# xandercai/JSPSR

Measured on AMD Instinct MI355X. Metric: Mpixels/sec fwd+bwd, JSPSR x8 on 512^2 DEM tiles, higher is better.
Workload: dtype bf16; 1 GPU; jspsr_r8_img_msk (image+mask guided, 43.87M params), 8 x 512x512 tiles per GPU, train step (fwd + L1/L2/Sobel loss + bwd + grad all-reduce + AdamW); storage policy: bf16 activations / gradients / MFMA operands, fp32 accumulation, BatchNorm statistics, master weights and optimizer, and the generator head (affinity logits + offsets) kept as fp32 planes; tiles_per_gpu=8, tile=512, global_tiles=8, parallelism=dp1, step_mode=eager

## Files before the change

jspsr_amd/csrc/elementwise.hip:

```cpp
#include "common.h"

#include <cstdlib>

namespace {

using namespace jspsr;

constexpr int TX = 64, TY = 4;

template <typename T> struct V;
template <> struct V<float> { static constexpr int N = 4; };
template <> struct V<__bf16> { static constexpr int N = 8; };

template <typename T, int N>
struct Pack { T v[N]; };

template <typename T>
__device__ __forceinline__ uint4 load_raw(const T* p) { return *reinterpret_cast<const uint4*>(p); }
template <typename T>
__device__ __forceinline__ void unpack(const uint4& raw, float (&f)[V<T>::N]) {
  if constexpr (sizeof(T) == 4) {
    f[0] = __uint_as_float(raw.x); f[1] = __uint_as_float(raw.y); f[2] = __uint_as_float(raw.z); f[3] = __uint_as_float(raw.w);
  } else {
    const unsigned w[4] = {raw.x, raw.y, raw.z, raw.w};
// ... 514 lines not shown
    for (int k = 0; k < 8; ++k) {
      const size_t o = ((size_t)b * chunks + r + k) * C + c;
      ps[k] = psum[o]; pm[k] = pmax[o]; pi[k] = pidx[o];
    }
#pragma unroll
    for (int k = 0; k < 8; ++k) {
      s += (double)ps[k];
      if (pm[k] > m || (pm[k] == m && pi[k] < ii)) { m = pm[k]; ii = pi[k]; }
    }
  }
  for (; r < chunks; ++r) {
    const size_t o = ((size_t)b * chunks + r) * C + c;
    s += (double)psum[o];
    if (pmax[o] > m || (pmax[o] == m && pidx[o] < ii)) { m = pmax[o]; ii = pidx[o]; }
  }
  avg[(size_t)b * C + c] = (float)(s / (double)npix);
  mx[(size_t)b * C + c] = m;
  amax[(size_t)b * C + c] = ii;
}

template <typename T>
__global__ __launch_bounds__(TX * TY) void gate_scale_kernel(const T* __restrict__ x, const float* __restrict__ s,
                                                            T* __restrict__ y, RedGeom g) {
  constexpr int N = V<T>::N;
  float sv[N];
  const int c0 = lane_map<N>(g).c;
  if (c0 < g.C) load_param<N>(s + (size_t)(blockIdx.x / g.chunks) * g.C + c0, sv);
  for_pixels_mlp<T, 1>(
      g, [&](long long pix, int c, uint4 (&raw)[1]) { raw[0] = load_raw<T>(x + (size_t)pix * g.C + c); },
      [&](long long, long long pix, int c, const uint4 (&raw)[1]) {
        float f[N];
        unpack<T>(raw[0], f);
#pragma unroll
        for (int k = 0; k < N; ++k) f[k] *= sv[k];
        store_vec<T>(y + (size_t)pix * g.C + c, f);
      });
}

template <typename T>
__global__ __launch_bounds__(TX * TY) void gate_bwd_reduce_kernel(const T* __restrict__ dy, const T* __restrict__ x,
                                                                 RedGeom g, float* __restrict__ partial) {
  constexpr int N = V<T>::N;
  reduce_pixels_mlp<T, 1, 2>(
      g, partial,
      [&](long long pix, int c, uint4 (&raw)[2]) {
        raw[0] = load_raw<T>(dy + (size_t)pix * g.C + c);
        raw[1] = load_raw<T>(x + (size_t)pix * g.C + c);
      },
      [&](long long, int, const uint4 (&raw)[2], float (&acc)[1][N]) {
        float d[N], xv[N];
        unpack<T>(raw[0], d);
        unpack<T>(raw[1], xv);
#pragma unroll
        for (int i = 0; i < N; ++i) acc[0][i] += d[i] * xv[i];
      });
}

__global__ void gate_bwd_finalize_kernel(const float* __restrict__ partial, int chunks, int C, float* __restrict__ ds) {
  const int c = blockIdx.x * blockDim.x + threadIdx.x, b = blockIdx.y;
  if (c >= C) return;
  double s = 0.0;
  int r = 0;
  for (; r + 8 <= chunks; r += 8) {
    float v[8];
#pragma unroll
    for (int k = 0; k < 8; ++k) v[k] = partial[((size_t)b * chunks + r + k) * C + c];
#pragma unroll
    for (int k = 0; k < 8; ++k) s += (double)v[k];
  }
  for (; r < chunks; ++r) s += (double)partial[((size_t)b * chunks + r) * C + c];
  ds[(size_t)b * C + c] = (float)s;
}

template <typename T>
__global__ __launch_bounds__(TX * TY) void gate_bwd_apply_kernel(const T* __restrict__ dy, const float* __restrict__ s,
                                                                const float* __restrict__ davg, const float* __restrict__ dmax,
                                                                const int* __restrict__ amax, T* __restrict__ dx, RedGeom g) {
  constexpr int N = V<T>::N;
  float sv[N], da[N], dm[N];
  int am[N];
  const int c0 = lane_map<N>(g).c;
  const float inv = 1.f / (float)g.npix;
  if (c0 < g.C) {
    const size_t o = (size_t)(blockIdx.x / g.chunks) * g.C + c0;
    load_param<N>(s + o, sv); load_param<N>(davg + o, da); load_param<N>(dmax + o, dm);
#pragma unroll
    for (int k = 0; k < N; ++k) { am[k] = amax[o + k]; da[k] *= inv; }
  }
  for_pixels_mlp<T, 1>(
      g, [&](long long pix, int c, uint4 (&raw)[1]) { raw[0] = load_raw<T>(dy + (size_t)pix * g.C + c); },
      [&](long long p, long long pix, int c, const uint4 (&raw)[1]) {
        float f[N];
        unpack<T>(raw[0], f);
#pragma unroll
        for (int k = 0; k < N; ++k) f[k] = f[k] * sv[k] + da[k] + (am[k] == (int)p ? dm[k] : 0.f);
        store_vec<T>(dx + (size_t)pix * g.C + c, f);
      });
}

int ew_blocks(long long total) {
  long long b = (total + 255) / 256;
  return (int)(b < 1 ? 1 : (b > 4096 ? 4096 : b));
}

int check_c(int dtype, int C, const char* what) {
  if (dtype != JSPSR_F32 && dtype != JSPSR_BF16) return fail(JSPSR_EINVAL, "%s: bad dtype", what);
  const int vec = dtype == JSPSR_F32 ? 4 : 8;
  if (C <= 0 || C % vec) return fail(JSPSR_EINVAL, "%s: C=%d must be a multiple of %d", what, C, vec);
  return JSPSR_OK;
}

}

#define DISPATCH(dtype, CALL)                    \
  do {                                           \
    if ((dtype) == JSPSR_F32) { using T = float; CALL; } else { using T = __bf16; CALL; } \
  } while (0)

extern "C" size_t jspsr_reduce_workspace_bytes(int dtype, int C, int nseg) {
  if (C <= 0 || nseg <= 0) return 0;
  const int vec = dtype == JSPSR_F32 ? 4 : 8;
  const RedGeom g = make_red(1LL << 40, nseg, C, vec);
  const size_t rows = (size_t)nseg * g.chunks;
  return (rows * 3 + 4) * (size_t)C * sizeof(float) + 64;
}

extern "C" int jspsr_bn_forward(int dtype, const void* x, int x_cs, int x_coff, const void* res, int r_cs, int r_coff,
                                void* y, int y_cs, int y_coff, const float* gamma, const float* beta,
                                float* running_mean, float* running_var, float momentum, float eps, int training,
                                int relu, float res_scale, float* save_mean, float* save_invstd, long long npix, int C,
                                const float* ext_partial, int ext_rows, const float* res_affine, float* affine_out,
                                void* workspace, jspsr_stream_t stream) {
  if (int e = check_c(dtype, C, "bn_forward")) return e;
  if (!x || (!y && !affine_out) || !gamma || !beta || !save_mean || !save_invstd || !workspace || npix <= 0)
    return fail(JSPSR_EINVAL, "bn_forward: null pointer or empty tensor");
  if (res_affine && !res) return fail(JSPSR_EINVAL, "bn_forward: res_affine without a residual operand");
  if (!training && (!running_mean || !running_var)) return fail(JSPSR_EINVAL, "bn_forward: eval mode needs running stats");
  const int vec = dtype == JSPSR_F32 ? 4 : 8;
  if (x_cs % vec || x_coff % vec || y_cs % vec || y_coff % vec || (res && (r_cs % vec || r_coff % vec)))
    return fail(JSPSR_EINVAL, "bn_forward: channel pitches/offsets must be multiples of %d", vec);
  hipStream_t s = static_cast<hipStream_t>(stream);
  float* ws = static_cast<float*>(workspace);
  float* scale = affine_out ? affine_out : ws;
  float* shift = affine_out ? affine_out + C : ws + C;
  float* partial = ws + 2 * C;
  int rows = 0;
  if (training && ext_partial) {
    if (ext_rows <= 0) return fail(JSPSR_EINVAL, "bn_forward: ext_rows must be positive");
    rows = ext_rows < 256 ? ext_rows : 256;
    if (ext_rows > 256) {
      hipLaunchKernelGGL(fold_rows_kernel, dim3(rows, (2 * C + 255) / 256), dim3(256), 0, s, ext_partial, ext_rows, 2 * C, rows, partial);
      if (int e = check_launch("bn_fold_rows")) return e;
    } else {
      (void)hipMemcpyAsync(partial, ext_partial, (size_t)ext_rows * 2 * C * sizeof(float), hipMemcpyDeviceToDevice, s);
    }
  } else if (training) {
    const RedGeom g = make_red(npix, 1, C, vec);
    rows = g.chunks;
    DISPATCH(dtype, hipLaunchKernelGGL(bn_stats_kernel<T>, red_grid(g, vec), dim3(TX, TY), 0, s,
                                       static_cast<const T*>(x), x_cs, x_coff, g, partial));
    if (int e = check_launch("bn_stats")) return e;
  }
  hipLaunchKernelGGL(bn_finalize_kernel, dim3((C + 3) / 4), dim3(256), 0, s, partial, rows, C, npix, gamma, beta,
                     running_mean, running_var, momentum, eps, training, save_mean, save_invstd, scale, shift);
  if (int e = check_launch("bn_finalize")) return e;
  if (!y) return JSPSR_OK;
  const RedGeom ga = make_red(npix, 1, C, vec);
#define BN_APPLY(R) DISPATCH(dtype, hipLaunchKernelGGL((bn_apply_kernel<T, R>), red_grid(ga, vec), dim3(TX, TY), 0, s,             \
                                     static_cast<const T*>(x), x_cs, x_coff, static_cast<const T*>(res), r_cs, r_coff,        \
                                     static_cast<T*>(y), y_cs, y_coff, scale, shift, res_affine, res_scale, relu, ga))
  if (res) { BN_APPLY(true); } else { BN_APPLY(false); }
#undef BN_APPLY
  return check_launch("bn_apply");
}

__global__ void bn_reduce_params_kernel(const float* __restrict__ gamma, const float* __restrict__ beta, const float* __restrict__ mean,
                                        const float* __restrict__ invstd, int C, float* __restrict__ par) {
  const int c = blockIdx.x * blockDim.x + threadIdx.x;
  if (c >= C) return;
  const float a = gamma[c] * invstd[c];
  par[c] = a;
  par[C + c] = beta[c] - a * mean[c];
  par[2 * C + c] = invstd[c];
  par[3 * C + c] = -mean[c] * invstd[c];
}

extern "C" int jspsr_bn_reduce_params(const float* gamma, const float* beta, const float* save_mean, const float* save_invstd, int C,
                                      float* par, jspsr_stream_t stream) {
  if (!gamma || !beta || !save_mean || !save_invstd || !par || C <= 0) return fail(JSPSR_EINVAL, "bn_reduce_params: bad arguments");
  hipLaunchKernelGGL(bn_reduce_params_kernel, dim3((C + 255) / 256), dim3(256), 0, static_cast<hipStream_t>(stream), gamma, beta,
                     save_mean, save_invstd, C, par);
  return check_launch("bn_reduce_params");
}

extern "C" int jspsr_bn_backward(int dtype, const void* dy, int dy_cs, int dy_coff, const void* y, int y_cs, int y_coff,
                                 const void* x, int x_cs, int x_coff, const float* gamma, const float* beta, const float* save_mean,
                                 const float* save_invstd, int training, int relu, float res_scale, void* dx, void* dres,
                                 float* dgamma, float* dbeta, int accumulate, long long npix, int C, void* workspace,
                                 const float* ext_partial, int ext_rows, jspsr_stream_t stream) {
  if (int e = check_c(dtype, C, "bn_backward")) return e;
  if (!dy || !x || !gamma || !save_mean || !save_invstd || !dx || !dgamma || !dbeta || !workspace || npix <= 0 ||
      (relu == 1 && !y) || (relu == 2 && !beta) || relu < 0 || relu > 2)
    return fail(JSPSR_EINVAL, "bn_backward: null pointer, empty tensor or bad relu mode");
  const int vec = dtype == JSPSR_F32 ? 4 : 8;
  if (dy_cs % vec || dy_coff % vec || x_cs % vec || x_coff % vec || (relu == 1 && (y_cs % vec || y_coff % vec)))
    return fail(JSPSR_EINVAL, "bn_backward: channel pitches/offsets must be multiples of %d", vec);
  hipStream_t s = static_cast<hipStream_t>(stream);
  float* ws = static_cast<float*>(workspace);
  float* coef = ws;
  float* partial = ws + 3 * C;
  const RedGeom g = make_red(npix, 1, C, vec);
#define BN_BWD_REDUCE(R) DISPATCH(dtype, hipLaunchKernelGGL((bn_bwd_reduce_kernel<T, R>), red_grid(g, vec), dim3(TX, TY), 0, s, \
                                     static_cast<const T*>(dy), dy_cs, dy_coff, static_cast<const T*>(y), y_cs, y_coff,     \
                                     static_cast<const T*>(x), x_cs, x_coff, save_mean, save_invstd, gamma, beta, g, partial))
  int rows = g.chunks;
  if (ext_partial) {
    if (ext_rows <= 0) return fail(JSPSR_EINVAL, "bn_backward: ext_rows must be positive");
    if (ext_rows > 1024) {
      rows = g.chunks < 1024 ? (g.chunks > 0 ? g.chunks : 1) : 1024;
      hipLaunchKernelGGL(fold_rows_kernel, dim3(rows, (2 * C + 255) / 256), dim3(256), 0, s, ext_partial, ext_rows, 2 * C, rows, partial);
      if (int e = check_launch("bn_fold_rows")) return e;
    } else {
      partial = const_cast<float*>(ext_partial);
      rows = ext_rows;
    }
  } else {
    if (relu == 0) { BN_BWD_REDUCE(0); } else if (relu == 1) { BN_BWD_REDUCE(1); } else { BN_BWD_REDUCE(2); }
    if (int e = check_launch("bn_bwd_reduce")) return e;
  }
#undef BN_BWD_REDUCE
  hipLaunchKernelGGL(bn_bwd_finalize_kernel, dim3((C + 3) / 4), dim3(256), 0, s, partial, rows, C, npix, gamma,
                     save_invstd, training, res_scale, accumulate, dgamma, dbeta, coef);
  if (int e = check_launch("bn_bwd_finalize")) return e;
#define BN_BWD_APPLY(R) DISPATCH(dtype, hipLaunchKernelGGL((bn_bwd_apply_kernel<T, R>), red_grid(g, vec), dim3(TX, TY), 0, s,  \
                                     static_cast<const T*>(dy), dy_cs, dy_coff, static_cast<const T*>(y), y_cs, y_coff,     \
                                     static_cast<const T*>(x), x_cs, x_coff, save_mean, save_invstd, gamma, beta, coef,     \
                                     static_cast<T*>(dx), static_cast<T*>(dres), g))
  if (relu == 0) { BN_BWD_APPLY(0); } else if (relu == 1) { BN_BWD_APPLY(1); } else { BN_BWD_APPLY(2); }
#undef BN_BWD_APPLY
  return check_launch("bn_bwd_apply");
}

extern "C" int jspsr_bn_fold(const float* gamma, const float* beta, const float* running_mean, const float* running_var,
                             float eps, float res_scale, int C, float* scale, float* shift, jspsr_stream_t stream) {
  if (!gamma || !beta || !running_mean || !running_var || !scale || !shift || C <= 0)
    return fail(JSPSR_EINVAL, "bn_fold: bad arguments");
  hipLaunchKernelGGL(bn_fold_kernel, dim3((C + 255) / 256), dim3(256), 0, static_cast<hipStream_t>(stream), gamma, beta,
                     running_mean, running_var, eps, res_scale, C, scale, shift);
  return check_launch("bn_fold");
}

extern "C" int jspsr_act_backward(int dtype, const void* dy, int dy_cs, int dy_coff, const void* y, int y_cs, int relu,
                                  void* dz, int dz_cs, float* dbias, long long npix, int C, void* workspace,
                                  jspsr_stream_t stream) {
  if (int e = check_c(dtype, C, "act_backward")) return e;
  if (!dy || (relu && !y) || !workspace || npix <= 0) return fail(JSPSR_EINVAL, "act_backward: null pointer or empty tensor");
  const int vec = dtype == JSPSR_F32 ? 4 : 8;
  if (dy_cs % vec || dy_coff % vec || (dz && dz_cs % vec) || (relu && (y_cs % vec || y_cs < C)))
    return fail(JSPSR_EINVAL, "act_backward: bad pitch");
  hipStream_t s = static_cast<hipStream_t>(stream);
  float* partial = static_cast<float*>(workspace);
  const RedGeom g = make_red(npix, 1, C, vec);
#define ACT_BWD(R) DISPATCH(dtype, hipLaunchKernelGGL((act_bwd_kernel<T, R>), red_grid(g, vec), dim3(TX, TY), 0, s, static_cast<const T*>(dy), \
                                     dy_cs, dy_coff, static_cast<const T*>(y), y_cs, relu, static_cast<T*>(dz), dz_cs, g, partial))
  if (relu) { ACT_BWD(true); } else { ACT_BWD(false); }
#undef ACT_BWD
  if (int e = check_launch("act_backward")) return e;
  if (dbias) {
    hipLaunchKernelGGL(sum_rows_kernel, dim3((C + 3) / 4), dim3(256), 0, s, partial, g.chunks, 1, 0, C, dbias);
    return check_launch("act_backward_bias");
  }
  return JSPSR_OK;
}

extern "C" int jspsr_gate_pool(int dtype, const void* x, int B, long long npix, int C, float* avg, float* mx, int* amax,
                               void* workspace, jspsr_stream_t stream) {
  if (int e = check_c(dtype, C, "gate_pool")) return e;
  if (!x || !avg || !mx || !amax || !workspace || B <= 0 || npix <= 0 || npix > 0x7fffffffLL)
    return fail(JSPSR_EINVAL, "gate_pool: bad arguments");
  const int vec = dtype == JSPSR_F32 ? 4 : 8;
  hipStream_t s = static_cast<hipStream_t>(stream);
  const RedGeom g = make_red(npix, B, C, vec);
  const size_t rows = (size_t)B * g.chunks;
  float* psum = static_cast<float*>(workspace);
  float* pmax = psum + rows * C;
  int* pidx = reinterpret_cast<int*>(pmax + rows * C);
  DISPATCH(dtype, hipLaunchKernelGGL(gate_pool_kernel<T>, red_grid(g, vec), dim3(TX, TY), 0, s, static_cast<const T*>(x), g,
                                     psum, pmax, pidx));
  if (int e = check_launch("gate_pool")) return e;
  hipLaunchKernelGGL(gate_pool_finalize_kernel, dim3((C + 255) / 256, B), dim3(256), 0, s, psum, pmax, pidx, g.chunks, C,
                     npix, avg, mx, amax);
  return check_launch("gate_pool_finalize");
}

extern "C" int jspsr_gate_scale(int dtype, const void* x, const float* s_, void* y, int B, long long npix, int C,
                                jspsr_stream_t stream) {
  if (int e = check_c(dtype, C, "gate_scale")) return e;
  if (!x || !s_ || !y || B <= 0 || npix <= 0) return fail(JSPSR_EINVAL, "gate_scale: bad arguments");
  const int vec = dtype == JSPSR_F32 ? 4 : 8;
  hipStream_t s = static_cast<hipStream_t>(stream);
  const RedGeom g = make_red(npix, B, C, vec);
  DISPATCH(dtype, hipLaunchKernelGGL(gate_scale_kernel<T>, red_grid(g, vec), dim3(TX, TY), 0, s,
                                     static_cast<const T*>(x), s_, static_cast<T*>(y), g));
  return check_launch("gate_scale");
}

extern "C" int jspsr_gate_backward_reduce(int dtype, const void* dy, const void* x, float* ds, int B, long long npix, int C,
                                          void* workspace, jspsr_stream_t stream) {
  if (int e = check_c(dtype, C, "gate_backward_reduce")) return e;
  if (!dy || !x || !ds || !workspace || B <= 0 || npix <= 0) return fail(JSPSR_EINVAL, "gate_backward_reduce: bad arguments");
  const int vec = dtype == JSPSR_F32 ? 4 : 8;
  hipStream_t s = static_cast<hipStream_t>(stream);
  const RedGeom g = make_red(npix, B, C, vec);
  float* partial = static_cast<float*>(workspace);
  DISPATCH(dtype, hipLaunchKernelGGL(gate_bwd_reduce_kernel<T>, red_grid(g, vec), dim3(TX, TY), 0, s,
                                     static_cast<const T*>(dy), static_cast<const T*>(x), g, partial));
  if (int e = check_launch("gate_backward_reduce")) return e;
  hipLaunchKernelGGL(gate_bwd_finalize_kernel, dim3((C + 255) / 256, B), dim3(256), 0, s, partial, g.chunks, C, ds);
  return check_launch("gate_backward_finalize");
}

extern "C" int jspsr_gate_backward_apply(int dtype, const void* dy, const float* s_, const float* davg, const float* dmax,
                                         const int* amax, void* dx, int B, long long npix, int C, jspsr_stream_t stream) {
  if (int e = check_c(dtype, C, "gate_backward_apply")) return e;
  if (!dy || !s_ || !davg || !dmax || !amax || !dx || B <= 0 || npix <= 0)
    return fail(JSPSR_EINVAL, "gate_backward_apply: bad arguments");
  const int vec = dtype == JSPSR_F32 ? 4 : 8;
  hipStream_t s = static_cast<hipStream_t>(stream);
  const RedGeom g = make_red(npix, B, C, vec);
  DISPATCH(dtype, hipLaunchKernelGGL(gate_bwd_apply_kernel<T>, red_grid(g, vec), dim3(TX, TY), 0, s,
                                     static_cast<const T*>(dy), s_, davg, dmax, amax, static_cast<T*>(dx), g));
  return check_launch("gate_backward_apply");
}

template <typename T>
__global__ __launch_bounds__(256) void nchw_to_nhwc_kernel(const float* __restrict__ src, T* __restrict__ dst, int C, long long HW,
                                                          long long npix, int Cpad) {
  constexpr int N = V<T>::N;
  for (long long p = blockIdx.x * 256LL + threadIdx.x; p < npix; p += (long long)gridDim.x * 256) {
    const long long b = p / HW, q = p - b * HW;
    const float* s = src + (size_t)b * C * HW + q;
    T* d = dst + (size_t)p * Cpad;
    for (int c0 = 0; c0 < Cpad; c0 += N) {
      float f[N];
#pragma unroll
      for (int i = 0; i < N; ++i) f[i] = c0 + i < C ? s[(size_t)(c0 + i) * HW] : 0.f;
      store_vec<T>(d + c0, f);
    }
  }
}

extern "C" int jspsr_nchw_to_nhwc(int dtype, const float* src, void* dst, int B, int C, int H, int W, int c_pad,
                                  jspsr_stream_t stream) {
  if (dtype != JSPSR_F32 && dtype != JSPSR_BF16) return fail(JSPSR_EINVAL, "nchw_to_nhwc: dtype must be JSPSR_F32 or JSPSR_BF16");
  const int vec = dtype == JSPSR_F32 ? 4 : 8;
  if (!src || !dst || B <= 0 || C <= 0 || H <= 0 || W <= 0 || c_pad < C || c_pad % vec)
    return fail(JSPSR_EINVAL, "nchw_to_nhwc: bad arguments (c_pad must be a multiple of %d and >= C)", vec);
  if (!aligned4(src) || !aligned16(dst)) return fail(JSPSR_EALIGN, "nchw_to_nhwc: src must be 4-byte, dst 16-byte aligned");
  const long long HW = (long long)H * W, npix = HW * B;
  const long long want = (npix + 255) / 256;
  const int blocks = (int)(want > 8192 ? 8192 : want);
  hipStream_t s = static_cast<hipStream_t>(stream);
  DISPATCH(dtype, hipLaunchKernelGGL(nchw_to_nhwc_kernel<T>, dim3(blocks), dim3(256), 0, s, src, static_cast<T*>(dst), C, HW, npix, c_pad));
  return check_launch("nchw_to_nhwc");
}

constexpr int GM_T = 256;

__global__ __launch_bounds__(GM_T) void gate_mlp_fwd_kernel(const float* __restrict__ avg, const float* __restrict__ mx,
                                                           const float* __restrict__ w1, const float* __restrict__ w2, int C, int Ch,
                                                           float* __restrict__ s, float* __restrict__ hid) {
  extern __shared__ float gm_lds[];
  const int b = blockIdx.x, tid = threadIdx.x, wave = tid >> 6, lane = tid & 63;
  const float* a = avg + (size_t)b * C;
  const float* m = mx + (size_t)b * C;
  for (int j = wave; j < Ch; j += GM_T / 64) {
    const float* w = w1 + (size_t)j * C;
    float da = 0.f, dm = 0.f;
    for (int c = lane; c < C; c += 64) { const float wv = w[c]; da += wv * a[c]; dm += wv * m[c]; }
#pragma unroll
    for (int d = 32; d > 0; d >>= 1) { da += __shfl_xor(da, d, 64); dm += __shfl_xor(dm, d, 64); }
    if (lane == 0) {
      const float ha = fmaxf(da, 0.f), hm = fmaxf(dm, 0.f);
      hid[((size_t)b * 2 + 0) * Ch + j] = ha;
      hid[((size_t)b * 2 + 1) * Ch + j] = hm;
      gm_lds[j] = ha + hm;
    }
  }
  __syncthreads();
  for (int c = tid; c < C; c += GM_T) {
    const float* w = w2 + (size_t)c * Ch;
    float z = 0.f;
    for (int j = 0; j < Ch; ++j) z += w[j] * gm_lds[j];
    s[(size_t)b * C + c] = 1.f / (1.f + expf(-z));
  }
}

__global__ __launch_bounds__(GM_T) void gate_mlp_bwd_kernel(const float* __restrict__ ds, const float* __restrict__ s,
                                                           const float* __restrict__ hid, const float* __restrict__ w1,
                                                           const float* __restrict__ w2, int C, int Ch, float* __restrict__ davg,
                                                           float* __restrict__ dmax, float* __restrict__ dzs, float* __restrict__ dhs) {
  extern __shared__ float gm_lds[];
  float* dz = gm_lds;
  float* dh = gm_lds + C;
  const int b = blockIdx.x, tid = threadIdx.x, wave = tid >> 6, lane = tid & 63;
  for (int c = tid; c < C; c += GM_T) {
    const float sv = s[(size_t)b * C + c], v = ds[(size_t)b * C + c] * sv * (1.f - sv);
    dz[c] = v;
    dzs[(size_t)b * C + c] = v;
  }
  __syncthreads();
  for (int j = wave; j < Ch; j += GM_T / 64) {
    float acc = 0.f;
    for (int c = lane; c < C; c += 64) acc += w2[(size_t)c * Ch + j] * dz[c];
#pragma unroll
    for (int d = 32; d > 0; d >>= 1) acc += __shfl_xor(acc, d, 64);
    if (lane == 0) {
      const float da = hid[((size_t)b * 2 + 0) * Ch + j] > 0.f ? acc : 0.f, dm = hid[((size_t)b * 2 + 1) * Ch + j] > 0.f ? acc : 0.f;
      dh[j] = da; dh[Ch + j] = dm;
      dhs[((size_t)b * 2 + 0) * Ch + j] = da;
      dhs[((size_t)b * 2 + 1) * Ch + j] = dm;
    }
  }
  __syncthreads();
  for (int c = tid; c < C; c += GM_T) {
    float ga = 0.f, gm = 0.f;
    for (int j = 0; j < Ch; ++j) { const float wv = w1[(size_t)j * C + c]; ga += wv * dh[j]; gm += wv * dh[Ch + j]; }
    davg[(size_t)b * C + c] = ga;
    dmax[(size_t)b * C + c] = gm;
  }
}

__global__ __launch_bounds__(GM_T) void gate_mlp_wgrad_kernel(const float* __restrict__ dzs, const float* __restrict__ dhs,
                                                             const float* __restrict__ hid, const float* __restrict__ avg,
                                                             const float* __restrict__ mx, int B, int C, int Ch,
                                                             float* __restrict__ dw1, float* __restrict__ dw2) {
  const long long n = (long long)C * Ch;
  for (long long i = blockIdx.x * (long long)GM_T + threadIdx.x; i < 2 * n; i += (long long)gridDim.x * GM_T) {
    if (i < n) {
      const int j = (int)(i / C), c = (int)(i - (long long)j * C);
      float g = 0.f;
      for (int b = 0; b < B; ++b)
        g += dhs[((size_t)b * 2 + 0) * Ch + j] * avg[(size_t)b * C + c] + dhs[((size_t)b * 2 + 1) * Ch + j] * mx[(size_t)b * C + c];
      dw1[i] = g;
    } else {
      const long long k = i - n;
      const int c = (int)(k / Ch), j = (int)(k - (long long)c * Ch);
      float g = 0.f;
      for (int b = 0; b < B; ++b) g += dzs[(size_t)b * C + c] * (hid[((size_t)b * 2 + 0) * Ch + j] + hid[((size_t)b * 2 + 1) * Ch + j]);
      dw2[k] = g;
    }
  }
}

extern "C" int jspsr_gate_mlp_forward(const float* avg, const float* mx, const float* w1, const float* w2, int B, int C, int Ch,
                                      float* s, float* hid, jspsr_stream_t stream) {
  if (!avg || !mx || !w1 || !w2 || !s || !hid || B <= 0 || C <= 0 || Ch <= 0 || Ch > 4096)
    return fail(JSPSR_EINVAL, "gate_mlp_forward: bad arguments");
  hipLaunchKernelGGL(gate_mlp_fwd_kernel, dim3(B), dim3(GM_T), Ch * sizeof(float), static_cast<hipStream_t>(stream), avg, mx, w1, w2,
                     C, Ch, s, hid);
  return check_launch("gate_mlp_forward");
}

extern "C" size_t jspsr_gate_mlp_backward_workspace_bytes(int B, int C, int Ch) {
  if (B <= 0 || C <= 0 || Ch <= 0) return 0;
  return ((size_t)B * C + (size_t)B * 2 * Ch) * sizeof(float);
}

extern "C" int jspsr_gate_mlp_backward(const float* ds, const float* s, const float* hid, const float* avg, const float* mx,
                                       const float* w1, const float* w2, int B, int C, int Ch, float* davg, float* dmax,
                                       float* dw1, float* dw2, void* workspace, jspsr_stream_t stream) {
  if (!ds || !s || !hid || !avg || !mx || !w1 || !w2 || !davg || !dmax || !dw1 || !dw2 || !workspace || B <= 0 || C <= 0 ||
      Ch <= 0 || (size_t)(C + 2 * Ch) * sizeof(float) > 64 * 1024)
    return fail(JSPSR_EINVAL, "gate_mlp_backward: bad arguments");
  float* dzs = static_cast<float*>(workspace);
  float* dhs = dzs + (size_t)B * C;
  hipStream_t st = static_cast<hipStream_t>(stream);
  hipLaunchKernelGGL(gate_mlp_bwd_kernel, dim3(B), dim3(GM_T), (C + 2 * Ch) * sizeof(float), st, ds, s, hid, w1, w2, C, Ch, davg, dmax,
                     dzs, dhs);
  if (int e = check_launch("gate_mlp_backward")) return e;
  const long long n2 = 2LL * C * Ch;
  const int blocks = (int)((n2 + GM_T - 1) / GM_T > 2048 ? 2048 : (n2 + GM_T - 1) / GM_T);
  hipLaunchKernelGGL(gate_mlp_wgrad_kernel, dim3(blocks), dim3(GM_T), 0, st, dzs, dhs, hid, avg, mx, B, C, Ch, dw1, dw2);
  return check_launch("gate_mlp_wgrad");
}
```

jspsr_amd/engine.py:

```python
from __future__ import annotations

import os

import torch

from . import kernels as K
from . import ops

_compute_dtype = torch.float32
_gate_sync = None
_offset_probe = None


class compute_dtype:

    def __init__(self, dtype):
        if dtype not in (torch.float32, torch.bfloat16):
            raise ValueError("compute dtype must be torch.float32 or torch.bfloat16")
        self.dtype = dtype

    def __enter__(self):
        global _compute_dtype
        self.prev, _compute_dtype = _compute_dtype, self.dtype

    def __exit__(self, *a):
        global _compute_dtype
        _compute_dtype = self.prev


def _gpu(x: torch.Tensor) -> torch.Tensor:
    if not x.is_cuda:
        raise RuntimeError("jspsr_amd runs on the GPU only: move the module and its inputs to cuda "
                           "(there is no CPU fallback; the CPU restatement lives in oracle/ for tests)")
    return x


def from_nchw(x: torch.Tensor) -> torch.Tensor:
    _gpu(x)
    B, C, H, W = x.shape
    e = K.epc(_compute_dtype)
    if x.dtype == torch.float32 and x.is_contiguous() and not (x.requires_grad and torch.is_grad_enabled()):
        return K.nchw_to_nhwc(x, _compute_dtype, (C + e - 1) // e * e)
    x = x.reshape(B, H, W, 1) if C == 1 else x.permute(0, 2, 3, 1)
    return ops.pad_channels(x.to(_compute_dtype), e).contiguous()


def to_nchw_f32(x: torch.Tensor) -> torch.Tensor:
    B, H, W, C = x.shape
    if C == 1:
        return x.float().reshape(B, 1, H, W)
    return x.permute(0, 3, 1, 2).float().contiguous()


SliceBuffer = ops.SliceBuffer


def conv2d(x, weight, bias=None, stride=1, padding=0, relu=False, dest=None):
    return ops.conv2d(x, weight, bias, stride, padding, relu, dest)


def conv_transpose2d(x, weight):
    return ops.conv_transpose2d(x, weight)


_nbt_pending = None


class count_batches:

    def __enter__(self):
        global _nbt_pending
        self.prev, _nbt_pending = _nbt_pending, []
        return self

    def __exit__(self, *a):
        global _nbt_pending
        todo, _nbt_pending = _nbt_pending, self.prev
        if todo and a[0] is None:
            seen = {}
            for t in todo:
                seen[id(t)] = (t, seen.get(id(t), (t, 0))[1] + 1)
            once = [t for t, k in seen.values() if k == 1]
            if once:
                torch._foreach_add_(once, 1)
            for t, k in seen.values():
                if k > 1:
                    t += k
        return False


def _count_batch(bn):
    if bn.training and bn.track_running_stats and bn.num_batches_tracked is not None:
        if _nbt_pending is not None:
            _nbt_pending.append(bn.num_batches_tracked)
        else:
            bn.num_batches_tracked += 1


def batch_norm(x, bn: torch.nn.BatchNorm2d, relu=False, residual=None, res_scale=1.0, partial=None, dest=None):
    training = bn.training or bn.running_mean is None
    _count_batch(bn)
    return ops.batch_norm(x, bn.weight, bn.bias, bn.running_mean, bn.running_var, bn.momentum, bn.eps, training,
                          relu, residual, res_scale, partial, dest)


def conv_bn(x, weight, bn: torch.nn.BatchNorm2d, stride=1, padding=0, relu=False, residual=None, res_scale=1.0, dest=None):
    if bn.training or bn.running_mean is None:
        y, st = ops.conv2d_with_stats(x, weight, stride, padding)
        return batch_norm(y, bn, relu, residual, res_scale, partial=st, dest=dest)
    if not torch.is_grad_enabled():
        return ops.conv_bn_infer(x, weight, bn.weight, bn.bias, _bn_state(bn), stride, padding, relu, residual,
                                 res_scale, dest)
    return batch_norm(ops.conv2d(x, weight, None, stride, padding), bn, relu, residual, res_scale, dest=dest)


def _bn_state(bn: torch.nn.BatchNorm2d):
    training = bn.training or bn.running_mean is None
    _count_batch(bn)
    return (bn.running_mean, bn.running_var, bn.momentum, bn.eps, training)


def res_unit(x, conv1, bn1, conv2, bn2, downsample, stride, scale, act, dest=None, grad_extra=None):
    bns = [_bn_state(bn1), _bn_state(bn2)]
    wd = gd = bd = None
    if downsample is not None:
        wd, gd, bd = downsample[0].weight, downsample[1].weight, downsample[1].bias
        bns.append(_bn_state(downsample[1]))
    return ops.res_unit(x, conv1.weight, bn1.weight, bn1.bias, conv2.weight, bn2.weight, bn2.bias, wd, gd, bd,
                        stride, scale, act, tuple(bns), dest, grad_extra)


def channel_gate(x, w1, w2):
    if _gate_sync is not None:
        avg, mx = _gate_sync.pool(x.contiguous())
        s = ops._gate_mlp(avg, mx, w1.detach().float(), w2.detach().float()).contiguous()
        return K.gate_scale(x.contiguous(), s)
    return ops.channel_gate(x, w1, w2)


def propagate_head(dem, head, w, b, scale=1.0):
    return ops.propagate_head(dem.contiguous(), head, w, b, scale)


planar_heads = os.environ.get("JSPSR_HEAD_PLANES", "1") != "0"


def heads_propagate(dem, feature, conv_weight, conv_offset, w, b, scale=1.0):
    dem = dem.contiguous()
    if planar_heads and ops.head_planes_ok(feature):
        planes = ops.head_planes(feature, conv_weight.weight, conv_weight.bias, conv_offset.weight, conv_offset.bias)
        if _offset_probe is not None:
            _offset_probe.append(planes[:, 9:].permute(0, 2, 3, 1))
        return ops.propagate_logits(dem, planes, w, b, scale)
    w_all, b_all = ops.merge_heads(conv_weight.weight, conv_weight.bias, conv_offset.weight, conv_offset.bias)
    head = conv2d(feature, w_all, b_all)
    if _offset_probe is not None:
        _offset_probe.append(ops.split_head(head)[1])
    return ops.propagate_head(dem, head, w, b, scale)


def conv_head1(x, weight, bias):
    return ops.conv_head1(x, weight, bias)


def cat(tensors):
    return torch.cat(tuple(tensors), 3)


def sigmoid(x):
    return torch.sigmoid(x)


def propagate(dem, weight, offset, w, b, scale=1.0):
    return ops.propagate(dem.contiguous(), weight.contiguous(), offset.contiguous(), w, b, scale)
```

jspsr_amd/ops.py:

```python
from __future__ import annotations

import collections
import os
import weakref

import torch

from . import _lib
from . import kernels as K


def _stream() -> int:
    return torch.cuda.current_stream().cuda_stream


def _need_gpu(*ts):
    for t in ts:
        if not t.is_cuda:
            raise RuntimeError("jspsr_amd ops run on the GPU only (got a CPU tensor); there is no CPU fallback")
        if t.dtype != torch.float32:
            raise TypeError(f"expected float32, got {t.dtype}")


def prop_forward_raw(dem, weight, offset, w, b, scale, out):
# ... 769 lines not shown
            aff1 = None
        if has_d:
            rmd, rvd, momd, epsd, trd = bns[2]
            wdd, gdd, bdd = wd.detach().contiguous(), gd.detach(), bd.detach()
            if fold_shortcut_bn:
                zd, r_aff, md, idd = conv_bn(x, wdd, 1, stride, 0, gdd, bdd, rmd, rvd, momd, epsd, trd, False, par=wd, stats_only=True)
                r = zd
            else:
                zd, r, md, idd = conv_bn(x, wdd, 1, stride, 0, gdd, bdd, rmd, rvd, momd, epsd, trd, False, par=wd)
                r_aff = None
        else:
            r_aff = None
            if stride != 1 or O != I:
                raise ValueError("res_unit: identity shortcut needs stride 1 and equal channel counts")
            wdd = gdd = bdd = zd = md = idd = None
            trd = False
            r = x
        out_v = dest[0].slice(dest[1], O, z1.shape[:3]) if dest is not None else None
        z2, out, m2, i2 = conv_bn(z1 if fuse1 else y1, w2d, 3, 1, 1, g2d, b2d, rm2, rv2, mom2, eps2, tr2, bool(act), r, float(scale),
                                  out_v, par=w2, res_affine=r_aff, in_affine=aff1)
        ctx.cfg = (stride, float(scale), bool(act), has_d, tr1, tr2, trd)
        ctx.wparams = tuple(p if isinstance(p, torch.nn.Parameter) else None for p in (w1, w2, wd))
        ctx.bparams = tuple(p if isinstance(p, torch.nn.Parameter) else None for p in (g1, b1, g2, b2, gd, bd))
        ctx.save_for_backward(x, w1d, g1d, b1d, z1, m1, i1, y1, w2d, g2d, b2d, z2, m2, i2, out if act else None,
                              wdd, gdd, bdd, zd, md, idd, aff1)
        return out

    @staticmethod
    def backward(ctx, dout):
        stride, scale, act, has_d, tr1, tr2, trd = ctx.cfg
        (x, w1, g1, b1, z1, m1, i1, y1, w2, g2, b2, z2, m2, i2, out, wd, gd, bd, zd, md, idd, aff1) = ctx.saved_tensors
        cdt = x.dtype
        B, H, W, Cin = x.shape
        O = w1.shape[0]
        dout = K.nhwc(dout)
        need_x = ctx.needs_input_grad[0]
        pg1, pb1, pg2, pb2, pgd, pbd = ctx.bparams
        sink2, sink1 = _bn_sink(pg2, pb2), _bn_sink(pg1, pb1)
        dz2, dres, dg2, db2 = K.bn_backward(dout, out, z2, g2, m2, i2, tr2, 1 if act else 0, scale,
                                            want_dres=(need_x or has_d), beta=b2, grads_into=sink2)
        if sink2 is not None:
            _bn_ready(pg2, pb2)
        if dres is None:
            dres = dout
        p1, p2, pd = ctx.wparams

        def wgrad2():
            if aff1 is not None:
                return _wgrad_async(p2, dz2, z1, O, O, 3, 3, 1, 1, x_affine=aff1, x_relu=True)
            return _wgrad_async(p2, dz2, y1, O, O, 3, 3, 1, 1)

        if not wgrad_after_dgrad:
            dW2 = wgrad2()
        Bz, Hz, Wz, _ = z1.shape
        part1 = None
        if bn_reduce_fused and tr1 and K.dgrad_reduce_ok(cdt, Bz, Hz, Wz, O, O, 3, 3, 1, 1) and z1.is_contiguous():
            par1 = K.bn_reduce_params(g1, b1, m1, i1)
            dy1, part1 = K.conv2d_dgrad(dz2, _packed(p2, w2, 1, O, cdt), z1.shape[1:3], 1, 1, red=(z1, par1))
        else:
            dy1 = K.conv2d_dgrad(dz2, _packed(p2, w2, 1, O, cdt), z1.shape[1:3], 1, 1)
        if wgrad_after_dgrad:
            dW2 = wgrad2()
        del dz2
        dz1, _, dg1, db1 = K.bn_backward(dy1, None, z1, g1, m1, i1, tr1, 2, 1.0, beta=b1, grads_into=sink1, ext_partial=part1)
        if sink1 is not None:
            _bn_ready(pg1, pb1)
        del dy1
        dW1 = None if wgrad_after_dgrad else _wgrad_async(p1, dz1, x, O, Cin, 3, 3, stride, 1)
        dWd = dgd = dbd = None
        side = dres
        deposit = None
        if isinstance(ctx.grad_extra, tuple):
            holder, off, n = ctx.grad_extra
            if holder.deferred is not None and has_d and need_x:
                cur = torch.cuda.current_stream()
                cur.wait_event(holder.deferred_event)
                deposit = holder.deferred.narrow(3, off, n)
                if tuple(deposit.shape) != tuple(x.shape):
                    raise RuntimeError(f"res_unit: parked gradient slice {tuple(deposit.shape)} does not match the input {tuple(x.shape)}")
                if deposit.dtype != x.dtype or not (deposit.is_contiguous() or K.is_slice(deposit)):
                    holder.pending_deposits -= 1
                    deposit = None
                else:
                    deposit.record_stream(cur)
            elif holder.deferred is not None:
                holder.pending_deposits -= 1
        extra = ctx.grad_extra.take_deferred() if (ctx.grad_extra is not None and not isinstance(ctx.grad_extra, tuple)) else deposit
        if extra is not None:
            extra = K.nhwc(extra)
            if tuple(extra.shape) != tuple(x.shape):
                raise RuntimeError(f"res_unit: deferred gradient {tuple(extra.shape)} does not match the input {tuple(x.shape)}")
            if not (has_d and need_x):
                side, extra = side + extra, None
        if has_d:
            sinkd = _bn_sink(pgd, pbd)
            dzd, _, dgd, dbd = K.bn_backward(dres, None, zd, gd, md, idd, trd, 0, 1.0, beta=bd, grads_into=sinkd)
            if sinkd is not None:
                _bn_ready(pgd, pbd)
            dWd = _wgrad_async(pd, dzd, x, O, Cin, 1, 1, stride, 0)
            side = K.conv2d_dgrad(dzd, _packed(pd, wd, 1, O, cdt), (H, W), stride, 0, addend=extra) if need_x else None
        dx = None
        if need_x and deposit is not None:
            K.conv2d_dgrad(dz1, _packed(p1, w1, 1, O, cdt), (H, W), stride, 1, addend=K.nhwc(side), out=deposit)
            ctx.grad_extra[0].deposit_events.append(torch.cuda.current_stream().record_event())
        elif need_x:
            dx = K.conv2d_dgrad(dz1, _packed(p1, w1, 1, O, cdt), (H, W), stride, 1, addend=K.nhwc(side))
        if wgrad_after_dgrad:
            dW1 = _wgrad_async(p1, dz1, x, O, Cin, 3, 3, stride, 1)
        return (dx, dW1, dg1, db1, dW2, dg2, db2, dWd, dgd, dbd, None, None, None, None, None, None)


def conv_bn_infer(x, weight, gamma, beta, bn, stride, pad, relu=False, res=None, res_scale=1.0, dest=None):
    x = K.nhwc(x)
    rm, rv, _, eps, training = bn
    if training or rm is None:
        raise RuntimeError("conv_bn_infer: BatchNorm must be in eval mode with running statistics")
    sc, sh = K.bn_fold(gamma.detach(), beta.detach(), rm, rv, eps, res_scale if res is not None else 1.0)
    O, I, KH, KW = weight.shape
    B, H, W, Cp = x.shape
    out = None
    if dest is not None:
        out = dest[0].slice(dest[1], O, (B, (H + 2 * pad - KH) // stride + 1, (W + 2 * pad - KW) // stride + 1))
    return K.conv2d_forward(x, _packed(weight, weight.detach().contiguous(), 0, Cp, x.dtype), sh, stride, pad, relu, out=out,
                            scale=sc, addend=K.nhwc(res) if res is not None else None)


def conv_transpose_bn_infer(x, weight, gamma, beta, bn, relu=True, dest=None):
    x = K.nhwc(x)
    rm, rv, _, eps, training = bn
    if training or rm is None:
        raise RuntimeError("conv_transpose_bn_infer: BatchNorm must be in eval mode with running statistics")
    I, O, KH, KW = weight.shape
    B, H, W, Cp = x.shape
    if Cp != I or KH != 3:
        raise ValueError("conv_transpose: only k3 s2 p1 op1 without channel padding is built")
    sc, sh = K.bn_fold(gamma.detach(), beta.detach(), rm, rv, eps, 1.0)
    out = dest[0].slice(dest[1], O, (B, 2 * H, 2 * W)) if dest is not None else None
    return K.conv2d_dgrad(x, _packed(weight, weight.detach().contiguous(), 1, Cp, x.dtype), (2 * H, 2 * W), 2, 1, bias=sh,
                          relu=relu, out=out, scale=sc)


def res_unit_infer(x, w1, g1, b1, w2, g2, b2, wd, gd, bd, stride, scale, act, bns, dest=None):
    y1 = conv_bn_infer(x, w1, g1, b1, bns[0], stride, 1, relu=True)
    r = conv_bn_infer(x, wd, gd, bd, bns[2], stride, 0) if wd is not None else x
    return conv_bn_infer(y1, w2, g2, b2, bns[1], 1, 1, relu=bool(act), res=r, res_scale=scale, dest=dest)


def res_unit(x, w1, g1, b1, w2, g2, b2, wd, gd, bd, stride, scale, act, bns, dest=None, grad_extra=None):
    if not torch.is_grad_enabled() and not any(b[4] for b in bns):
        return res_unit_infer(x, w1, g1, b1, w2, g2, b2, wd, gd, bd, stride, scale, act, bns, dest)
    return _ResUnit.apply(x, w1, g1, b1, w2, g2, b2, wd, gd, bd, stride, scale, act, bns, dest, grad_extra)


def _gate_mlp(avg, mx, w1, w2):
    f = torch.nn.functional
    h = lambda v: f.linear(f.relu(f.linear(v, w1.flatten(1))), w2.flatten(1))
    return torch.sigmoid(h(avg) + h(mx))


class _ChannelGate(torch.autograd.Function):

    @staticmethod
    def forward(ctx, x, w1, w2):
        x = x.contiguous()
        avg, mx, amax = K.gate_pool(x)
        w1f, w2f = w1.detach().float().flatten(1).contiguous(), w2.detach().float().flatten(1).contiguous()
        s, hid = K.gate_mlp_forward(avg, mx, w1f, w2f)
        y = K.gate_scale(x, s)
        ctx.save_for_backward(x, avg, mx, amax, s, hid, w1f, w2f)
        ctx.wshapes = (w1.shape, w2.shape, w1.dtype, w2.dtype)
        return y

    @staticmethod
    def backward(ctx, dy):
        x, avg, mx, amax, s, hid, w1f, w2f = ctx.saved_tensors
        dy = dy.contiguous()
        ds = K.gate_backward_reduce(dy, x)
        davg, dmax, dw1, dw2 = K.gate_mlp_backward(ds, s, hid, avg, mx, w1f, w2f)
        dx = K.gate_backward_apply(dy, s, davg, dmax, amax)
        s1, s2, t1, t2 = ctx.wshapes
        return dx, dw1.reshape(s1).to(t1), dw2.reshape(s2).to(t2)


def channel_gate(x, w1, w2):
    return _ChannelGate.apply(x, w1, w2)
```

Before: 34.29 Mpixel/s.

## Parallelize channel-gate MLP over batch×hidden and fuse dgrad with wgrad launch

Splits the per-batch channel-gate MLP kernels into wave-per-(batch,hidden) kernels with unrolled loads, so the small MLP spreads across many more compute units instead of B blocks. The backward input-grad pass and the weight-grad pass now run in one merged launch, and the inference gate path calls the custom kernel instead of a chain of torch linear ops. BN statistics also read external partial sums in place rather than copying them first. In exchange there is an extra forward launch and a B ≤ 65535 limit, and in the backward hidden pass the lanes with j==0 write dz redundantly.

```diff
diff --git a/jspsr_amd/csrc/elementwise.hip b/jspsr_amd/csrc/elementwise.hip
--- a/jspsr_amd/csrc/elementwise.hip
+++ b/jspsr_amd/csrc/elementwise.hip
@@ -690,7 +690,7 @@
       hipLaunchKernelGGL(fold_rows_kernel, dim3(rows, (2 * C + 255) / 256), dim3(256), 0, s, ext_partial, ext_rows, 2 * C, rows, partial);
       if (int e = check_launch("bn_fold_rows")) return e;
     } else {
-      (void)hipMemcpyAsync(partial, ext_partial, (size_t)ext_rows * 2 * C * sizeof(float), hipMemcpyDeviceToDevice, s);
+      partial = const_cast<float*>(ext_partial);
     }
   } else if (training) {
     const RedGeom g = make_red(npix, 1, C, vec);
@@ -904,77 +904,124 @@
 }
 
 constexpr int GM_T = 256;
-
-__global__ __launch_bounds__(GM_T) void gate_mlp_fwd_kernel(const float* __restrict__ avg, const float* __restrict__ mx,
-                                                           const float* __restrict__ w1, const float* __restrict__ w2, int C, int Ch,
-                                                           float* __restrict__ s, float* __restrict__ hid) {
-  extern __shared__ float gm_lds[];
-  const int b = blockIdx.x, tid = threadIdx.x, wave = tid >> 6, lane = tid & 63;
+constexpr int GM_U = 8;
+
+
+__global__ __launch_bounds__(GM_T) void gate_mlp_hidden_kernel(const float* __restrict__ avg, const float* __restrict__ mx,
+                                                              const float* __restrict__ w1, int B, int C, int Ch,
+                                                              float* __restrict__ hid) {
+  const int u = blockIdx.x * (GM_T / 64) + (threadIdx.x >> 6), lane = threadIdx.x & 63;
+  if (u >= B * Ch) return;
+  const int b = u / Ch, j = u - b * Ch;
   const float* a = avg + (size_t)b * C;
   const float* m = mx + (size_t)b * C;
-  for (int j = wave; j < Ch; j += GM_T / 64) {
-    const float* w = w1 + (size_t)j * C;
-    float da = 0.f, dm = 0.f;
-    for (int c = lane; c < C; c += 64) { const float wv = w[c]; da += wv * a[c]; dm += wv * m[c]; }
-#pragma unroll
-    for (int d = 32; d > 0; d >>= 1) { da += __shfl_xor(da, d, 64); dm += __shfl_xor(dm, d, 64); }
-    if (lane == 0) {
-      const float ha = fmaxf(da, 0.f), hm = fmaxf(dm, 0.f);
-      hid[((size_t)b * 2 + 0) * Ch + j] = ha;
-      hid[((size_t)b * 2 + 1) * Ch + j] = hm;
-      gm_lds[j] = ha + hm;
-    }
-  }
+  const float* w = w1 + (size_t)j * C;
+  float da = 0.f, dm = 0.f;
+  int c = lane;
+  for (; c + (GM_U - 1) * 64 < C; c += GM_U * 64) {
+    float wv[GM_U], av[GM_U], mv[GM_U];
+#pragma unroll
+    for (int k = 0; k < GM_U; ++k) { wv[k] = w[c + k * 64]; av[k] = a[c + k * 64]; mv[k] = m[c + k * 64]; }
+#pragma unroll
+    for (int k = 0; k < GM_U; ++k) { da = fmaf(wv[k], av[k], da); dm = fmaf(wv[k], mv[k], dm); }
+  }
+  for (; c < C; c += 64) { const float wv = w[c]; da = fmaf(wv, a[c], da); dm = fmaf(wv, m[c], dm); }
+#pragma unroll
+  for (int d = 32; d > 0; d >>= 1) { da += __shfl_xor(da, d, 64); dm += __shfl_xor(dm, d, 64); }
+  if (lane == 0) {
+    hid[((size_t)b * 2 + 0) * Ch + j] = fmaxf(da, 0.f);
+    hid[((size_t)b * 2 + 1) * Ch + j] = fmaxf(dm, 0.f);
+  }
+}
+
+__global__ __launch_bounds__(64) void gate_mlp_out_kernel(const float* __restrict__ hid, const float* __restrict__ w2, int C, int Ch,
+                                                         float* __restrict__ s) {
+  extern __shared__ float gm_lds[];
+  const int b = blockIdx.y, c = blockIdx.x * 64 + threadIdx.x;
+  for (int j = threadIdx.x; j < Ch; j += 64) gm_lds[j] = hid[((size_t)b * 2 + 0) * Ch + j] + hid[((size_t)b * 2 + 1) * Ch + j];
   __syncthreads();
-  for (int c = tid; c < C; c += GM_T) {
-    const float* w = w2 + (size_t)c * Ch;
-    float z = 0.f;
-    for (int j = 0; j < Ch; ++j) z += w[j] * gm_lds[j];
-    s[(size_t)b * C + c] = 1.f / (1.f + expf(-z));
-  }
-}
-
-__global__ __launch_bounds__(GM_T) void gate_mlp_bwd_kernel(const float* __restrict__ ds, const float* __restrict__ s,
-                                                           const float* __restrict__ hid, const float* __restrict__ w1,
-                                                           const float* __restrict__ w2, int C, int Ch, float* __restrict__ davg,
-                                                           float* __restrict__ dmax, float* __restrict__ dzs, float* __restrict__ dhs) {
+  if (c >= C) return;
+  const float* w = w2 + (size_t)c * Ch;
+  float z = 0.f;
+  int j = 0;
+  for (; j + 2 * GM_U <= Ch; j += 2 * GM_U) {
+    float wv[2 * GM_U];
+#pragma unroll
+    for (int k = 0; k < 2 * GM_U; ++k) wv[k] = w[j + k];
+#pragma unroll
+    for (int k = 0; k < 2 * GM_U; ++k) z = fmaf(wv[k], gm_lds[j + k], z);
+  }
+  for (; j < Ch; ++j) z = fmaf(w[j], gm_lds[j], z);
+  s[(size_t)b * C + c] = 1.f / (1.f + expf(-z));
+}
+
+__global__ __launch_bounds__(GM_T) void gate_mlp_bwd_hidden_kernel(const float* __restrict__ ds, const float* __restrict__ s,
+                                                                  const float* __restrict__ hid, const float* __restrict__ w2,
+                                                                  int B, int C, int Ch, float* __restrict__ dzs,
+                                                                  float* __restrict__ dhs) {
+  const int u = blockIdx.x * (GM_T / 64) + (threadIdx.x >> 6), lane = threadIdx.x & 63;
+  if (u >= B * Ch) return;
+  const int b = u / Ch, j = u - b * Ch;
+  const float* sp = s + (size_t)b * C;
+  const float* dp = ds + (size_t)b * C;
+  float* zp = dzs + (size_t)b * C;
+  float acc = 0.f;
+  int c = lane;
+  for (; c + (GM_U - 1) * 64 < C; c += GM_U * 64) {
+    float wv[GM_U], sv[GM_U], dv[GM_U];
+#pragma unroll
+    for (int k = 0; k < GM_U; ++k) { wv[k] = w2[(size_t)(c + k * 64) * Ch + j]; sv[k] = sp[c + k * 64]; dv[k] = dp[c + k * 64]; }
+#pragma unroll
+    for (int k = 0; k < GM_U; ++k) {
+      const float v = dv[k] * sv[k] * (1.f - sv[k]);
+      acc = fmaf(wv[k], v, acc);
+      if (j == 0) zp[c + k * 64] = v;
+    }
+  }
+  for (; c < C; c += 64) {
+    const float sv = sp[c], v = dp[c] * sv * (1.f - sv);
+    acc = fmaf(w2[(size_t)c * Ch + j], v, acc);
+    if (j == 0) zp[c] = v;
+  }
+#pragma unroll
+  for (int d = 32; d > 0; d >>= 1) acc += __shfl_xor(acc, d, 64);
+  if (lane == 0) {
+    dhs[((size_t)b * 2 + 0) * Ch + j] = hid[((size_t)b * 2 + 0) * Ch + j] > 0.f ? acc : 0.f;
+    dhs[((size_t)b * 2 + 1) * Ch + j] = hid[((size_t)b * 2 + 1) * Ch + j] > 0.f ? acc : 0.f;
+  }
+}
+
+__global__ __launch_bounds__(GM_T) void gate_mlp_bwd_out_kernel(const float* __restrict__ dzs, const float* __restrict__ dhs,
+                                                               const float* __restrict__ hid, const float* __restrict__ avg,
+                                                               const float* __restrict__ mx, const float* __restrict__ w1, int B,
+                                                               int C, int Ch, int nbx, float* __restrict__ davg,
+                                                               float* __restrict__ dmax, float* __restrict__ dw1,
+                                                               float* __restrict__ dw2) {
   extern __shared__ float gm_lds[];
-  float* dz = gm_lds;
-  float* dh = gm_lds + C;
-  const int b = blockIdx.x, tid = threadIdx.x, wave = tid >> 6, lane = tid & 63;
-  for (int c = tid; c < C; c += GM_T) {
-    const float sv = s[(size_t)b * C + c], v = ds[(size_t)b * C + c] * sv * (1.f - sv);
-    dz[c] = v;
-    dzs[(size_t)b * C + c] = v;
-  }
-  __syncthreads();
-  for (int j = wave; j < Ch; j += GM_T / 64) {
-    float acc = 0.f;
-    for (int c = lane; c < C; c += 64) acc += w2[(size_t)c * Ch + j] * dz[c];
-#pragma unroll
-    for (int d = 32; d > 0; d >>= 1) acc += __shfl_xor(acc, d, 64);
-    if (lane == 0) {
-      const float da = hid[((size_t)b * 2 + 0) * Ch + j] > 0.f ? acc : 0.f, dm = hid[((size_t)b * 2 + 1) * Ch + j] > 0.f ? acc : 0.f;
-      dh[j] = da; dh[Ch + j] = dm;
-      dhs[((size_t)b * 2 + 0) * Ch + j] = da;
-      dhs[((size_t)b * 2 + 1) * Ch + j] = dm;
-    }
-  }
-  __syncthreads();
-  for (int c = tid; c < C; c += GM_T) {
+  const int tid = threadIdx.x;
+  if ((int)blockIdx.x < nbx * B) {
+    const int b = blockIdx.x / nbx, c = (blockIdx.x - b * nbx) * GM_T + tid;
+    for (int j = tid; j < 2 * Ch; j += GM_T) gm_lds[j] = dhs[(size_t)b * 2 * Ch + j];
+    __syncthreads();
+    if (c >= C) return;
+    const float* dh = gm_lds;
     float ga = 0.f, gm = 0.f;
-    for (int j = 0; j < Ch; ++j) { const float wv = w1[(size_t)j * C + c]; ga += wv * dh[j]; gm += wv * dh[Ch + j]; }
+    int j = 0;
+    for (; j + GM_U <= Ch; j += GM_U) {
+      float wv[GM_U];
+#pragma unroll
+      for (int k = 0; k < GM_U; ++k) wv[k] = w1[(size_t)(j + k) * C + c];
+#pragma unroll
+      for (int k = 0; k < GM_U; ++k) { ga = fmaf(wv[k], dh[j + k], ga); gm = fmaf(wv[k], dh[Ch + j + k], gm); }
+    }
+    for (; j < Ch; ++j) { const float wv = w1[(size_t)j * C + c]; ga = fmaf(wv, dh[j], ga); gm = fmaf(wv, dh[Ch + j], gm); }
     davg[(size_t)b * C + c] = ga;
     dmax[(size_t)b * C + c] = gm;
-  }
-}
-
-__global__ __launch_bounds__(GM_T) void gate_mlp_wgrad_kernel(const float* __restrict__ dzs, const float* __restrict__ dhs,
-                                                             const float* __restrict__ hid, const float* __restrict__ avg,
-                                                             const float* __restrict__ mx, int B, int C, int Ch,
-                                                             float* __restrict__ dw1, float* __restrict__ dw2) {
-  const long long n = (long long)C * Ch;
-  for (long long i = blockIdx.x * (long long)GM_T + threadIdx.x; i < 2 * n; i += (long long)gridDim.x * GM_T) {
+    return;
+  }
+  const long long n = (long long)C * Ch, first = (long long)(blockIdx.x - nbx * B) * GM_T + tid;
+  const long long stride = (long long)(gridDim.x - nbx * B) * GM_T;
+  for (long long i = first; i < 2 * n; i += stride) {
     if (i < n) {
       const int j = (int)(i / C), c = (int)(i - (long long)j * C);
       float g = 0.f;
@@ -993,10 +1040,12 @@
 
 extern "C" int jspsr_gate_mlp_forward(const float* avg, const float* mx, const float* w1, const float* w2, int B, int C, int Ch,
                                       float* s, float* hid, jspsr_stream_t stream) {
-  if (!avg || !mx || !w1 || !w2 || !s || !hid || B <= 0 || C <= 0 || Ch <= 0 || Ch > 4096)
+  if (!avg || !mx || !w1 || !w2 || !s || !hid || B <= 0 || C <= 0 || Ch <= 0 || Ch > 4096 || B > 65535)
     return fail(JSPSR_EINVAL, "gate_mlp_forward: bad arguments");
-  hipLaunchKernelGGL(gate_mlp_fwd_kernel, dim3(B), dim3(GM_T), Ch * sizeof(float), static_cast<hipStream_t>(stream), avg, mx, w1, w2,
-                     C, Ch, s, hid);
+  hipStream_t st = static_cast<hipStream_t>(stream);
+  hipLaunchKernelGGL(gate_mlp_hidden_kernel, dim3((B * Ch + GM_T / 64 - 1) / (GM_T / 64)), dim3(GM_T), 0, st, avg, mx, w1, B, C, Ch, hid);
+  if (int e = check_launch("gate_mlp_hidden")) return e;
+  hipLaunchKernelGGL(gate_mlp_out_kernel, dim3((C + 63) / 64, B), dim3(64), Ch * sizeof(float), st, hid, w2, C, Ch, s);
   return check_launch("gate_mlp_forward");
 }
 
@@ -1014,11 +1063,13 @@
   float* dzs = static_cast<float*>(workspace);
   float* dhs = dzs + (size_t)B * C;
   hipStream_t st = static_cast<hipStream_t>(stream);
-  hipLaunchKernelGGL(gate_mlp_bwd_kernel, dim3(B), dim3(GM_T), (C + 2 * Ch) * sizeof(float), st, ds, s, hid, w1, w2, C, Ch, davg, dmax,
+  hipLaunchKernelGGL(gate_mlp_bwd_hidden_kernel, dim3((B * Ch + GM_T / 64 - 1) / (GM_T / 64)), dim3(GM_T), 0, st, ds, s, hid, w2, B, C, Ch,
                      dzs, dhs);
   if (int e = check_launch("gate_mlp_backward")) return e;
   const long long n2 = 2LL * C * Ch;
+  const int nbx = (C + GM_T - 1) / GM_T;
   const int blocks = (int)((n2 + GM_T - 1) / GM_T > 2048 ? 2048 : (n2 + GM_T - 1) / GM_T);
-  hipLaunchKernelGGL(gate_mlp_wgrad_kernel, dim3(blocks), dim3(GM_T), 0, st, dzs, dhs, hid, avg, mx, B, C, Ch, dw1, dw2);
+  hipLaunchKernelGGL(gate_mlp_bwd_out_kernel, dim3(nbx * B + blocks), dim3(GM_T), 2 * Ch * sizeof(float), st, dzs, dhs, hid, avg, mx, w1,
+                     B, C, Ch, nbx, davg, dmax, dw1, dw2);
   return check_launch("gate_mlp_wgrad");
 }
diff --git a/jspsr_amd/engine.py b/jspsr_amd/engine.py
--- a/jspsr_amd/engine.py
+++ b/jspsr_amd/engine.py
@@ -133,7 +133,8 @@
 def channel_gate(x, w1, w2):
     if _gate_sync is not None:
         avg, mx = _gate_sync.pool(x.contiguous())
-        s = ops._gate_mlp(avg, mx, w1.detach().float(), w2.detach().float()).contiguous()
+        s, _ = K.gate_mlp_forward(avg.float().contiguous(), mx.float().contiguous(), w1.detach().float().flatten(1).contiguous(),
+                                  w2.detach().float().flatten(1).contiguous())
         return K.gate_scale(x.contiguous(), s)
     return ops.channel_gate(x, w1, w2)
 
diff --git a/jspsr_amd/ops.py b/jspsr_amd/ops.py
--- a/jspsr_amd/ops.py
+++ b/jspsr_amd/ops.py
@@ -945,12 +945,6 @@
     return _ResUnit.apply(x, w1, g1, b1, w2, g2, b2, wd, gd, bd, stride, scale, act, bns, dest, grad_extra)
 
 
-def _gate_mlp(avg, mx, w1, w2):
-    f = torch.nn.functional
-    h = lambda v: f.linear(f.relu(f.linear(v, w1.flatten(1))), w2.flatten(1))
-    return torch.sigmoid(h(avg) + h(mx))
-
-
 class _ChannelGate(torch.autograd.Function):
 
     @staticmethod
```

Measured after the change: 34.76 Mpixel/s, median of 6. +1.4%, better.
